# jeffreyhorn/network_flow_solver

Hardware: AMD Instinct MI355X
Metric: pivots/sec + arcs-priced/sec (value = arcs-priced/sec; pivots_per_sec alongside) on netgen_8-style DIMACS (higher is better)
Workload: dtype int64; 1 GPU; netgen_8_08a(synthetic,x1): 256 nodes / 2048 arcs; pricing=full-scan Dantzig, step=one pivot (price + ratio test + tree/potential update), parallelism=1 GPU, sweeps=full (every arc priced every pivot)

## Files before the change

__graft_entry__.py:

```python

from __future__ import annotations

import os
import re
import subprocess
import sys
from pathlib import Path

ROOT = Path(__file__).resolve().parent
PKG = ROOT / "network_flow_solver_amd"
CSRC = PKG / "csrc"
LIB = PKG / "libmcf_hip.so"
CERT_HOST_LIB = PKG / "libmcf_certify_host.so"
REPAIR_HOST_LIB = PKG / "libmcf_repair_host.so"
FARKAS_HOST_LIB = PKG / "libmcf_farkas_host.so"
TOPOLOGY_HOST_LIB = PKG / "libmcf_topology_host.so"
RANGES_HOST_LIB = PKG / "libmcf_ranges_host.so"
FLOW_RANGES_HOST_LIB = PKG / "libmcf_flow_ranges_host.so"
DUAL_HOST_LIB = PKG / "libmcf_dual_host.so"
APPLY_PATHS_HOST_LIB = PKG / "libmcf_apply_paths_host.so"
SMALL_REDUCE_HOST_LIB = PKG / "libmcf_small_reduce_host.so"

if str(ROOT) not in sys.path:
    sys.path.insert(0, str(ROOT))


def _hipcc() -> str:
    for cand in (os.environ.get("HIPCC"), "/opt/rocm/bin/hipcc", "hipcc"):
        if cand and (os.path.isabs(cand) and os.path.exists(cand) or not os.path.isabs(cand)):
            return cand
    return "hipcc"


def _needs_rebuild(target: Path, sources) -> bool:
    if not target.exists():
        return True
    t = target.stat().st_mtime
    return any(Path(s).stat().st_mtime > t for s in sources)


def build_hip(force: bool = False) -> Path:
    sources = [CSRC / "mcf_engine.hip", CSRC / "mcf_passes_dev.h", CSRC / "mcf_passes_host.h", CSRC / "mcf_core.h", CSRC / "mcf_host.h",
               ROOT / "include" / "mcf.h"]
    if force or _needs_rebuild(LIB, sources):
        cmd = [_hipcc(), "--offload-arch=gfx950", "-O3", "-std=c++17", "-fPIC", "-shared",
               "-o", str(LIB), str(CSRC / "mcf_engine.hip")]
        subprocess.run(cmd, check=True, cwd=str(CSRC))
    return LIB


def build_certify_host(force: bool = False) -> Path:
    src = CSRC / "mcf_certify_host.cpp"
    if force or _needs_rebuild(CERT_HOST_LIB, [src, CSRC / "mcf_core.h"]):
        subprocess.run(["g++", "-O2", "-std=c++17", "-fPIC", "-shared", "-o", str(CERT_HOST_LIB), str(src)], check=True, cwd=str(CSRC))
    return CERT_HOST_LIB


def build_repair_host(force: bool = False) -> Path:
    src = CSRC / "mcf_repair_host.cpp"
    if force or _needs_rebuild(REPAIR_HOST_LIB, [src, CSRC / "mcf_core.h", CSRC / "mcf_host.h"]):
        subprocess.run(["g++", "-O2", "-std=c++17", "-fPIC", "-shared", "-o", str(REPAIR_HOST_LIB), str(src)], check=True, cwd=str(CSRC))
    return REPAIR_HOST_LIB


def build_farkas_host(force: bool = False) -> Path:
    src = CSRC / "mcf_farkas_host.cpp"
    if force or _needs_rebuild(FARKAS_HOST_LIB, [src, CSRC / "mcf_core.h"]):
        subprocess.run(["g++", "-O2", "-std=c++17", "-fPIC", "-shared", "-o", str(FARKAS_HOST_LIB), str(src)], check=True, cwd=str(CSRC))
    return FARKAS_HOST_LIB


def build_topology_host(force: bool = False) -> Path:
    src = CSRC / "mcf_topology_host.cpp"
    if force or _needs_rebuild(TOPOLOGY_HOST_LIB, [src, CSRC / "mcf_core.h", CSRC / "mcf_host.h"]):
        subprocess.run(["g++", "-O2", "-std=c++17", "-fPIC", "-shared", "-o", str(TOPOLOGY_HOST_LIB), str(src)], check=True, cwd=str(CSRC))
    return TOPOLOGY_HOST_LIB


def build_ranges_host(force: bool = False) -> Path:
    src = CSRC / "mcf_ranges_host.cpp"
    if force or _needs_rebuild(RANGES_HOST_LIB, [src, CSRC / "mcf_core.h"]):
        subprocess.run(["g++", "-O2", "-std=c++17", "-fPIC", "-shared", "-o", str(RANGES_HOST_LIB), str(src)], check=True, cwd=str(CSRC))
    return RANGES_HOST_LIB


def build_flow_ranges_host(force: bool = False) -> Path:
    src = CSRC / "mcf_flow_ranges_host.cpp"
    if force or _needs_rebuild(FLOW_RANGES_HOST_LIB, [src, CSRC / "mcf_core.h"]):
        subprocess.run(["g++", "-O2", "-std=c++17", "-fPIC", "-shared", "-o", str(FLOW_RANGES_HOST_LIB), str(src)], check=True, cwd=str(CSRC))
    return FLOW_RANGES_HOST_LIB


def build_dual_host(force: bool = False) -> Path:
    src = CSRC / "mcf_dual_host.cpp"
    if force or _needs_rebuild(DUAL_HOST_LIB, [src, CSRC / "mcf_core.h", CSRC / "mcf_host.h", ROOT / "include" / "mcf.h"]):
        subprocess.run(["g++", "-O2", "-std=c++17", "-fPIC", "-shared", "-o", str(DUAL_HOST_LIB), str(src)], check=True, cwd=str(CSRC))
    return DUAL_HOST_LIB


def build_apply_paths_host(force: bool = False) -> Path:
    src = CSRC / "mcf_apply_paths_host.cpp"
    if force or _needs_rebuild(APPLY_PATHS_HOST_LIB, [src, CSRC / "mcf_core.h", CSRC / "mcf_host.h"]):
        subprocess.run(["g++", "-O2", "-std=c++17", "-fPIC", "-shared", "-o", str(APPLY_PATHS_HOST_LIB), str(src)], check=True, cwd=str(CSRC))
    return APPLY_PATHS_HOST_LIB


def build_small_reduce_host(force: bool = False) -> Path:
    src = CSRC / "mcf_small_reduce_host.cpp"
    if force or _needs_rebuild(SMALL_REDUCE_HOST_LIB, [src, CSRC / "mcf_core.h"]):
        subprocess.run(["g++", "-O2", "-std=c++17", "-fPIC", "-shared", "-o", str(SMALL_REDUCE_HOST_LIB), str(src)], check=True, cwd=str(CSRC))
    return SMALL_REDUCE_HOST_LIB


def declared_symbols() -> list[str]:
    text = (ROOT / "include" / "mcf.h").read_text()
    text = re.sub(r"/\*.*?\*/", "", text, flags=re.S)
    names = re.findall(r"\b(mcf_[a-z0-9_]+)\s*\(", text)
    return sorted(set(n for n in names if n != "mcf_progress_cb"))


def build() -> None:
    build_hip()
    import oracle

    oracle.build()
    oracle.build_emul()
    build_certify_host()
    build_repair_host()
    build_farkas_host()
    build_topology_host()
    build_ranges_host()
    build_flow_ranges_host()
    build_dual_host()
    build_apply_paths_host()
    build_small_reduce_host()
    import ctypes

    lib = ctypes.CDLL(str(LIB))
    missing = [s for s in declared_symbols() if not hasattr(lib, s)]
    if missing:
        raise RuntimeError(f"libmcf_hip.so lacks symbols declared in include/mcf.h: {missing}")
    import network_flow_solver_amd


def smoke() -> None:
    import numpy as np

    build_hip()
    import oracle
    from network_flow_solver_amd import engine, generators

    if engine.device_count() <= 0:
        raise RuntimeError("smoke() needs a GPU: no HIP device visible")
    inst = generators.netgen_style(256, 2048, seed=7)
    ref = oracle.solve_soa(inst, "dantzig")
    for rule in (engine.RULE_DANTZIG, engine.RULE_DEVEX_BLOCK, engine.RULE_CANDIDATE_LIST):
        with engine.McfEngine(inst.n, inst.tail, inst.head, inst.cost, inst.cap, inst.supply, rule=rule,
                              device=0) as eng:
            eng.solve()
            res = eng.result()
        assert res.status == ref["status"] == "optimal", (res.status, ref["status"])
        assert res.objective == int(round(ref["objective"])), (res.objective, ref["objective"])
        bal = inst.supply.astype(np.int64).copy()
        np.subtract.at(bal, inst.tail, res.flow)
        np.add.at(bal, inst.head, res.flow)
        assert not bal.any()
        rc = inst.cost + res.potential[inst.tail] - res.potential[inst.head]
        assert (rc[(res.flow > 0) & (res.flow < inst.cap)] == 0).all()
        assert (rc[(res.flow == 0) & (inst.cap > 0)] >= 0).all() and (rc[(res.flow == inst.cap) & (inst.cap > 0)] <= 0).all()
        print(f"smoke ok: rule={rule} objective={res.objective} pivots={res.stats['pivots']} "
              f"(oracle {ref['iterations']} pivots)")


if __name__ == "__main__":
    build()
    if len(sys.argv) > 1 and sys.argv[1] == "smoke":
        smoke()
```

network_flow_solver_amd/csrc/mcf_core.h:

```cpp
#pragma once
#include <stdint.h>

#if defined(__HIPCC__)
#define MCF_HD __host__ __device__ __forceinline__
#else
#define MCF_HD inline
#endif

#define MCF_INF ((int64_t)1 << 60)

#if defined(__HIP_DEVICE_COMPILE__)
#define mcf_double_bits(x) ((int64_t)__double_as_longlong(x))
#else
static inline int64_t mcf_double_bits(double x) { int64_t k; __builtin_memcpy(&k, &x, 8); return k; }
#endif

#if defined(__HIP_DEVICE_COMPILE__)
#define MCF_TEAM_BARRIER() __syncthreads()
#define MCF_ATOMIC_MIN64(p, x) atomicMin(reinterpret_cast<long long*>(p), (long long)(x))
#define MCF_ATOMIC_MIN32(p, x) atomicMin(reinterpret_cast<int*>(p), (int)(x))
#define MCF_ATOMIC_MAX32(p, x) atomicMax(reinterpret_cast<int*>(p), (int)(x))
#define MCF_ATOMIC_ADD32(p, x) atomicAdd(reinterpret_cast<int*>(p), (int)(x))
#define MCF_ATOMIC_MAX64(p, x) atomicMax(reinterpret_cast<long long*>(p), (long long)(x))
#define MCF_ATOMIC_OR32(p, x) atomicOr(reinterpret_cast<int*>(p), (int)(x))
// ... 6 lines not shown
#define MCF_ATOMIC_ADD32(p, x) mcf_host_fetch_add32((p), (x))
#define MCF_ATOMIC_MAX64(p, x) do { if ((int64_t)(x) > *(p)) *(p) = (int64_t)(x); } while (0)
#define MCF_ATOMIC_OR32(p, x) do { *(p) |= (int32_t)(x); } while (0)
#endif

enum McfStatus : int32_t {
    MCF_RUNNING = 0,
    MCF_OPTIMAL = 1,
    MCF_PIVOT_LIMIT = 2,
    MCF_UNBOUNDED = 3,
    MCF_INTERNAL_ERROR = 4
};

#define MCF_RULE_DANTZIG 0
#ifndef MCF_RULE_DEVEX_BLOCK
#define MCF_RULE_DEVEX_BLOCK 1
#endif
#ifndef MCF_RULE_CANDIDATE_LIST
#define MCF_RULE_CANDIDATE_LIST 2
#endif

#if defined(__HIPCC__)
template <int CTRL, int ROW_MASK>
__device__ __forceinline__ int64_t mcf_dpp_max_step(int64_t x) {
    const int lo = (int)(uint32_t)x, hi = (int)(uint32_t)((uint64_t)x >> 32);
    const int olo = __builtin_amdgcn_update_dpp(lo, lo, CTRL, ROW_MASK, 0xf, false);
    const int ohi = __builtin_amdgcn_update_dpp(hi, hi, CTRL, ROW_MASK, 0xf, false);
    const int64_t o = (int64_t)(((uint64_t)(uint32_t)ohi << 32) | (uint32_t)olo);
    return o > x ? o : x;
}
__device__ __forceinline__ int64_t mcf_wave_max64(int64_t x) {
    x = mcf_dpp_max_step<0xB1, 0xf>(x);
    x = mcf_dpp_max_step<0x4E, 0xf>(x);
    x = mcf_dpp_max_step<0x141, 0xf>(x);
    x = mcf_dpp_max_step<0x140, 0xf>(x);
    x = mcf_dpp_max_step<0x142, 0xa>(x);
    x = mcf_dpp_max_step<0x143, 0xc>(x);
    const uint32_t lo = (uint32_t)__builtin_amdgcn_readlane((int)(uint32_t)x, 63);
    const uint32_t hi = (uint32_t)__builtin_amdgcn_readlane((int)(uint32_t)((uint64_t)x >> 32), 63);
    return (int64_t)(((uint64_t)hi << 32) | lo);
}
template <int CTRL, int ROW_MASK>
__device__ __forceinline__ uint32_t mcf_dpp_min_u32_step(uint32_t x) {
    const uint32_t o = (uint32_t)__builtin_amdgcn_update_dpp((int)0xffffffffu, (int)x, CTRL, ROW_MASK, 0xf, false);
    return o < x ? o : x;
}
template <int CTRL, int ROW_MASK>
__device__ __forceinline__ uint32_t mcf_dpp_max_u32_step(uint32_t x) {
    const uint32_t o = (uint32_t)__builtin_amdgcn_update_dpp(0, (int)x, CTRL, ROW_MASK, 0xf, false);
    return o > x ? o : x;
}
__device__ __forceinline__ uint32_t mcf_wave_min_u32(uint32_t x) {
    x = mcf_dpp_min_u32_step<0xB1, 0xf>(x);
    x = mcf_dpp_min_u32_step<0x4E, 0xf>(x);
    x = mcf_dpp_min_u32_step<0x141, 0xf>(x);
    x = mcf_dpp_min_u32_step<0x140, 0xf>(x);
    x = mcf_dpp_min_u32_step<0x142, 0xa>(x);
    x = mcf_dpp_min_u32_step<0x143, 0xc>(x);
    return (uint32_t)__builtin_amdgcn_readlane((int)x, 63);
}
__device__ __forceinline__ uint32_t mcf_wave_max_u32(uint32_t x) {
    x = mcf_dpp_max_u32_step<0xB1, 0xf>(x);
    x = mcf_dpp_max_u32_step<0x4E, 0xf>(x);
    x = mcf_dpp_max_u32_step<0x141, 0xf>(x);
    x = mcf_dpp_max_u32_step<0x140, 0xf>(x);
    x = mcf_dpp_max_u32_step<0x142, 0xa>(x);
    x = mcf_dpp_max_u32_step<0x143, 0xc>(x);
    return (uint32_t)__builtin_amdgcn_readlane((int)x, 63);
}
#endif

MCF_HD bool mcf_ratio_narrow_ok(int64_t r) { return r == MCF_INF || (uint64_t)r <= 0xfffffffeull; }
MCF_HD uint32_t mcf_ratio_key32(int64_t r) { return r == MCF_INF ? 0xffffffffu : (uint32_t)r; }
MCF_HD int64_t mcf_ratio_unkey32(uint32_t k) { return k == 0xffffffffu ? MCF_INF : (int64_t)k; }
template <bool LAST>
MCF_HD void mcf_ratio_take(int64_t mn, uint64_t mask, int32_t base, int64_t& d, int32_t& k) {
    if (LAST ? mn <= d : mn < d) {
        d = mn;
        k = base + (LAST ? 63 - __builtin_clzll((unsigned long long)mask) : __builtin_ctzll((unsigned long long)mask));
    }
}
MCF_HD uint32_t mcf_argmax_viol(uint64_t packed) { return (uint32_t)(packed >> 32); }
MCF_HD uint32_t mcf_argmax_second(uint64_t packed, uint32_t vmx) { return mcf_argmax_viol(packed) == vmx ? (uint32_t)packed : 0u; }

#if defined(MCF_STAMPS) && defined(__HIPCC__)
__shared__ unsigned long long mcf_stamp_acc[24];
__shared__ unsigned long long mcf_stamp_last;
#define MCF_PSTAMP(slot)                                                     \
    do {                                                                      \
        if (threadIdx.x == 0) {                                               \
            const unsigned long long now_ = __builtin_amdgcn_s_memtime();     \
            mcf_stamp_acc[slot] += now_ - mcf_stamp_last;                     \
            mcf_stamp_last = now_;                                            \
        }                                                                     \
    } while (0)
#else
#define MCF_PSTAMP(slot) do {} while (0)
#endif

struct alignas(16) McfNode {
    int32_t parent;
    int32_t pred;
    int32_t size;
    int32_t depth;
};

struct alignas(16) McfArcW {
    int64_t cap;
    int64_t flow;
};

struct alignas(16) McfCand {
    int64_t key;
    int64_t arc;
};

struct alignas(16) McfCandX {
    int64_t rc;
    int64_t arc;
    int32_t tail, head;
    int32_t state;
    int32_t pad;
};

#define MCF_NUM_BUCKETS 8

#define MCF_GRANULES 64
#define MCF_WLIST_CAP 1024
#define MCF_DEVEX_RESET_SWAPS 64
#define MCF_TUNER_MAX_ARCS 16384
#define MCF_DIR_FLAG (1 << 30)
struct McfDevex {
    int32_t gran[MCF_NUM_BUCKETS][MCF_GRANULES + 1];
    int32_t gtot[MCF_GRANULES + 1];
    int32_t wlist[MCF_WLIST_CAP];
};

struct McfSeg {
    int32_t dst, src, len;
    int32_t ddepth;
};

struct McfCtx {
    int32_t status;
    int32_t unbounded_arc;
    int64_t pivots;
    int64_t degenerate;
    int64_t bound_flips;
    int64_t max_pivots;
    int64_t arcs_priced;
    int64_t nodes_moved;
    int64_t subtree_nodes;
    int64_t cycle_arcs;
    int64_t block_size;
    int64_t block_index;
    int32_t empty_blocks;
    int32_t num_blocks;
    int32_t block_granules;
    int32_t auto_tune;
    int32_t tn_total, tn_degenerate;
    int64_t tn_last_adapt;
    int32_t swaps_since_reset;
    int32_t wlist_n;
    int32_t wreset;
    int32_t devex_cyclic;
    int32_t max_granules;
// ... 1850 lines not shown
```

network_flow_solver_amd/csrc/mcf_engine.hip:

```cpp
#include <hip/hip_runtime.h>

#include <algorithm>
#include <cerrno>
#include <chrono>
#include <cstdio>
#include <cstdlib>
#include <cstring>
#include <mutex>
#include <new>
#include <string>
#include <vector>

#include "../../include/mcf.h"
#include "mcf_core.h"
#include "mcf_host.h"

namespace {

constexpr int kPriceThreads = 256;
constexpr int kPivotThreads = 1024;
constexpr int kReduceThreads = 256;
constexpr int kMidMaxNodes = 1536;
constexpr int kMidMaxArcsPerPivot = MCF_TUNER_MAX_ARCS + 1024;
constexpr int64_t kIncrementalMinArcs = (int64_t)1 << 22;
// ... 1200 lines not shown
template <bool MARK>
__global__ __launch_bounds__(kRcupdThreads) void k_rcupd(McfView g) {
    McfView v = g;
    if (!MARK) v.dirty = nullptr;
    const McfCtx c = *v.ctx;
    if (!c.apply) return;
    rcupd_pass(v, c, (int64_t)blockIdx.x * (kRcupdThreads / 16) + (threadIdx.x >> 4), (int64_t)gridDim.x * (kRcupdThreads / 16), threadIdx.x & 15);
}

__global__ __launch_bounds__(kApplyThreads) void k_apply(McfView v) {
    const McfCtx c = *v.ctx;
    if (!c.apply) return;
    const int xb = v.candx ? kCandxBlocks : 0;
    const int nb = (int)gridDim.x - xb;
    if ((int)blockIdx.x >= nb) { candx_pass(v, c, ((int)blockIdx.x - nb) * kApplyThreads + (int)threadIdx.x, xb * kApplyThreads); return; }
    apply_pass(v, c, (int64_t)blockIdx.x * kApplyThreads + threadIdx.x, (int64_t)nb * kApplyThreads);
}

__device__ __forceinline__ int swap01(int x) { return __builtin_amdgcn_update_dpp(x, x, 0xB1, 0xf, 0xf, false); }

__device__ __forceinline__ bool pivot_climb_2lanes(const McfView& v, McfCycle* out) {
    const McfCtx* c = v.ctx;
    const int side = threadIdx.x & 1;
    const int32_t* pcur = c->cur ? v.posbuf[1] : v.posbuf[0];
    int32_t node = side ? c->pv_second : c->pv_first;
    McfNode rec = v.node[node];
    int32_t pos = pcur[node];
    const McfNode rec0 = rec;
    const int32_t pos0 = pos;
    int32_t* const path = side ? v.path2 : v.path1;
    int32_t* const ppos = side ? v.ppos2 : v.ppos1;
    McfNode* const recs = side ? v.rec2 : v.rec1;
    int64_t d = MCF_INF;
    int32_t k = -1, n = 0, trips = 0;
    bool ok = true;
    for (;;) {
        const int32_t onode = swap01(node), odepth = swap01(rec.depth);
        if (node == onode) break;
        if (rec.depth >= odepth) {
            const McfNode nrec = v.node[rec.parent];
            const int32_t npos = pcur[rec.parent];
            const McfArcW a = v.arcw[rec.pred >> 1];
            const bool loses = ((rec.pred & 1) != 0) != (side != 0);
            const int64_t r = loses ? a.flow : (a.cap >= MCF_INF ? MCF_INF : a.cap - a.flow);
            if (side ? r <= d : r < d) { d = r; k = n; }
            path[n] = node;
            recs[n] = rec;
            ppos[n] = pos;
            ++n;
            node = rec.parent;
            rec = nrec;
            pos = npos;
        }
        if (++trips > v.n_nodes) { ok = false; break; }
    }
    const int32_t od_lo = swap01((int)(uint32_t)d), od_hi = swap01((int)(uint32_t)((uint64_t)d >> 32));
    const int32_t ok2 = swap01(k), on2 = swap01(n), opos0 = swap01(pos0);
    McfNode orec0;
    orec0.parent = swap01(rec0.parent); orec0.pred = swap01(rec0.pred); orec0.size = swap01(rec0.size); orec0.depth = swap01(rec0.depth);
    if (side == 0) {
        out->d1 = d; out->k1 = k; out->n1 = n;
        out->d2 = (int64_t)(((uint64_t)(uint32_t)od_hi << 32) | (uint32_t)od_lo); out->k2 = ok2; out->n2 = on2;
        out->u = node; out->w = node; out->pu = pos; out->pw = pos; out->ru = rec; out->rw = rec;
        out->p0u = pos0; out->p0w = opos0; out->r0u = rec0; out->r0w = orec0;
        out->small = 0;
    }
    return ok;
}

struct SmallLayout {
    uint32_t tail, head, cost, orig, state, weight, arcw, pi, node, order0, order1, pos0, pos1, path1, path2, ppos1, ppos2, rec1, rec2, seg, scratch, ctx, total;
};

constexpr int kSmallMaxLds = 156 * 1024;
constexpr int kSmallCycleMaxNodes = 1024;

#if defined(MCF_SMALL_LDS_SWEEP)
constexpr bool kRegSweep = false;
#else
constexpr bool kRegSweep = true;
#endif
template <int THREADS> struct SmallScalarControl { static constexpr bool value = THREADS > 256; };
template <int THREADS> struct SmallRegArcs { static constexpr int value = THREADS <= 256 ? 10 : (THREADS <= 512 ? 5 : 3); };

template <int THREADS>
__device__ __forceinline__ void copy_words(void* dst, const void* src, uint32_t bytes) {
    const uint32_t n = bytes >> 2;
    const int32_t* s = static_cast<const int32_t*>(src);
    int32_t* d = static_cast<int32_t*>(dst);
    for (uint32_t i = threadIdx.x; i < n; i += THREADS) d[i] = s[i];
}

#ifdef MCF_STAMPS
#define STAMP(slot)                                                                       \
    do {                                                                                  \
        if (threadIdx.x == 0) {                                                           \
            const unsigned long long now_ = __builtin_amdgcn_s_memtime();                 \
            stamps_[slot] += now_ - last_;                                                \
            last_ = now_;                                                                 \
        }                                                                                 \
    } while (0)
#else
#define STAMP(slot) do {} while (0)
#endif
#ifdef MCF_STAMPS
#define MCF_LAST_WAVE_BEGIN() const unsigned long long lw0_ = __builtin_amdgcn_s_memtime()
#define MCF_LAST_WAVE_STAMP() do { last_wave_ += __builtin_amdgcn_s_memtime() - lw0_; } while (0)
#else
#define MCF_LAST_WAVE_BEGIN() do {} while (0)
#define MCF_LAST_WAVE_STAMP() do {} while (0)
#endif

struct SmallCycleAcc {
    int32_t c1[16], c2[16];
};
#if defined(MCF_SMALL_JOIN)
template <int THREADS> struct SmallSearchJoin { static constexpr bool value = true; };
#else
template <int THREADS> struct SmallSearchJoin { static constexpr bool value = THREADS != 256; };
#endif

#if defined(MCF_SMALL_RATIO64)
constexpr bool kRatioNarrow = false;
#else
constexpr bool kRatioNarrow = true;
#endif
template <bool LAST>
__device__ __forceinline__ void small_ratio_side(const int64_t* res, int32_t n, int64_t* d_out, int32_t* k_out) {
    const int32_t lane = (int32_t)(threadIdx.x & 63);
    int64_t d = MCF_INF;
    int32_t k = -1;
    if (kRatioNarrow) {
        const int64_t r0 = lane < n ? res[lane] : MCF_INF;
        bool wide = !mcf_ratio_narrow_ok(r0);
        for (int32_t i = 64 + lane; i < n; i += 64) wide |= !mcf_ratio_narrow_ok(res[i]);
        if (__ballot(wide) == 0) {
            for (int32_t base = 0; base < n; base += 64) {
                const int32_t i = base + lane;
                const uint32_t key = mcf_ratio_key32(base == 0 ? r0 : (i < n ? res[i] : MCF_INF));
                const uint32_t mn = mcf_wave_min_u32(key);
                const uint64_t mask = __ballot(i < n && key == mn);
                mcf_ratio_take<LAST>(mcf_ratio_unkey32(mn), mask, base, d, k);
            }
            *d_out = d; *k_out = k;
            return;
        }
    }
    for (int32_t base = 0; base < n; base += 64) {
        const int32_t i = base + lane;
        const int64_t r = i < n ? res[i] : INT64_MAX;
        const int64_t mn = -mcf_wave_max64(-r);
        const uint64_t mask = __ballot(r == mn);
        mcf_ratio_take<LAST>(mn, mask, base, d, k);
    }
    *d_out = d; *k_out = k;
}

#if defined(MCF_SMALL_TWO_BRANCHES)
template <int THREADS> struct SmallSearchOneBranch { static constexpr bool value = false; };
#else
template <int THREADS> struct SmallSearchOneBranch { static constexpr bool value = THREADS == 256; };
#endif

template <int THREADS>
__device__ __forceinline__ void small_cycle_parallel(const McfView& v, SmallCycleAcc& A, int64_t* scratch, McfCycle& cy) {
    constexpr bool kScalar = SmallScalarControl<THREADS>::value;
// ... 262 lines not shown
    const uint32_t m_padb = m_pad4 >> 2;
    const uint32_t N = (uint32_t)g.n_nodes;
    const uint32_t arcw_b = (uint32_t)(g.m + N - 1) * 16u;
    McfView v = g;
    v.tail = reinterpret_cast<const int32_t*>(smem + L.tail);
    v.head = reinterpret_cast<const int32_t*>(smem + L.head);
    v.cost = reinterpret_cast<const int32_t*>(smem + L.cost);
    v.orig = reinterpret_cast<const int32_t*>(smem + L.orig);
    v.state = reinterpret_cast<int8_t*>(smem + L.state);
    v.weight = g.weight ? reinterpret_cast<float*>(smem + L.weight) : nullptr;
    v.arcw = reinterpret_cast<McfArcW*>(smem + L.arcw);
    v.pi = reinterpret_cast<int64_t*>(smem + L.pi);
    v.node = reinterpret_cast<McfNode*>(smem + L.node);
    v.order[0] = reinterpret_cast<int32_t*>(smem + L.order0);
    v.order[1] = reinterpret_cast<int32_t*>(smem + L.order1);
    v.path1 = reinterpret_cast<int32_t*>(smem + L.path1);
    v.path2 = reinterpret_cast<int32_t*>(smem + L.path2);
    v.ppos1 = reinterpret_cast<int32_t*>(smem + L.ppos1);
    v.ppos2 = reinterpret_cast<int32_t*>(smem + L.ppos2);
    v.rec1 = reinterpret_cast<McfNode*>(smem + L.rec1);
    v.rec2 = reinterpret_cast<McfNode*>(smem + L.rec2);
    v.seg = reinterpret_cast<McfSeg*>(smem + L.seg);
    v.ctx = reinterpret_cast<McfCtx*>(smem + L.ctx);
    v.posbuf[0] = reinterpret_cast<int32_t*>(smem + L.pos0);
    v.posbuf[1] = reinterpret_cast<int32_t*>(smem + L.pos1);
    v.psz[0] = nullptr;
    v.psz[1] = nullptr;
    v.reach = nullptr;
    v.bmeta[0] = nullptr; v.bmeta[1] = nullptr; v.candx = nullptr; v.dirty = nullptr; v.dirty_hdr = nullptr;
    v.rcache = nullptr; v.adj_off = nullptr;
    if constexpr (FRONT && kFrontNoDevex) { v.weight = nullptr; v.dx = nullptr; }

    copy_words<THREADS>(smem + L.tail, g.tail, m_pad4);
    copy_words<THREADS>(smem + L.head, g.head, m_pad4);
    copy_words<THREADS>(smem + L.cost, g.cost, m_pad4);
    copy_words<THREADS>(smem + L.orig, g.orig, m_pad4);
    copy_words<THREADS>(smem + L.state, g.state, m_padb);
    if (v.weight) copy_words<THREADS>(smem + L.weight, g.weight, m_pad4);
    copy_words<THREADS>(smem + L.arcw, g.arcw, arcw_b);
    copy_words<THREADS>(smem + L.pi, g.pi, N * 8u);
    copy_words<THREADS>(smem + L.node, g.node, N * 16u);
    copy_words<THREADS>(smem + L.order0, g.order[0], N * 4u);
    copy_words<THREADS>(smem + L.order1, g.order[1], N * 4u);
    copy_words<THREADS>(smem + L.pos0, g.posbuf[0], N * 4u);
    copy_words<THREADS>(smem + L.pos1, g.posbuf[1], N * 4u);
    copy_words<THREADS>(smem + L.ctx, g.ctx, (uint32_t)sizeof(McfCtx));
    __syncthreads();
    STAMP(0);

    McfCtx* const c = v.ctx;
    if (threadIdx.x == 0) arm_ctx(c, cap);
    __shared__ int32_t s_gran[MCF_NUM_BUCKETS][MCF_GRANULES + 1];
    const bool devex = !FRONT && rule == MCF_RULE_DEVEX_BLOCK && g.dx;
    if (devex) {
        for (int q = threadIdx.x; q < MCF_NUM_BUCKETS * (MCF_GRANULES + 1); q += THREADS)
            (&s_gran[0][0])[q] = (&g.dx->gran[0][0])[q];
    } else if (threadIdx.x < MCF_NUM_BUCKETS) {
        s_gran[threadIdx.x][0] = (int32_t)g.bucket_off[threadIdx.x];
        s_gran[threadIdx.x][MCF_GRANULES] = (int32_t)g.bucket_off[threadIdx.x + 1];
    }
    const bool listing = !FRONT && rule == MCF_RULE_CANDIDATE_LIST;
    __shared__ int64_t s_lk[MCF_NUM_BUCKETS], s_la[MCF_NUM_BUCKETS];
    if (listing && threadIdx.x < MCF_NUM_BUCKETS) { s_lk[threadIdx.x] = list[threadIdx.x].key; s_la[threadIdx.x] = list[threadIdx.x].arc; }
    __syncthreads();
    __shared__ int32_t s_gsum[MCF_GRANULES + 1];
    if (threadIdx.x <= MCF_GRANULES && (devex || threadIdx.x == 0 || threadIdx.x == MCF_GRANULES)) {
        int32_t sum = 0;
        for (int x = 0; x < MCF_NUM_BUCKETS; ++x) sum += s_gran[x][threadIdx.x];
        s_gsum[threadIdx.x] = sum;
    }
    __syncthreads();
    constexpr bool kScalar = SmallScalarControl<THREADS>::value;
    const int64_t priced_all = uni32<kScalar>(s_gsum[MCF_GRANULES] - s_gsum[0]);

    constexpr int kPer = THREADS / MCF_NUM_BUCKETS;
    constexpr int kReg = SmallRegArcs<THREADS>::value;
    static_assert(kPer == 32 || kPer % 64 == 0, "a head bucket's lanes are half a wave or whole waves");
    const int px = threadIdx.x / kPer, pl = threadIdx.x % kPer;
    const int sweep = FRONT ? (int)kSweepPlain
                            : (devex ? kSweepDevex : (rule != MCF_RULE_DEVEX_BLOCK && v.key_mode == MCF_KEY_PLAIN ? kSweepPlain : kSweepGeneric));
    int32_t r_tail[kReg], r_head[kReg], r_cost[kReg], r_orig[kReg];
    uint32_t r_info[kReg];
    int32_t r_n = 0;
    const int32_t r_lo = s_gran[px][0] + pl, r_hi = s_gran[px][MCF_GRANULES];
#pragma unroll
    for (int k = 0; k < kReg; ++k) {
        const int32_t i = r_lo + k * kPer;
        const bool on = kRegSweep && sweep == kSweepPlain && i < r_hi;
        r_tail[k] = on ? v.tail[i] : 0; r_head[k] = on ? v.head[i] : 0; r_cost[k] = on ? v.cost[i] : 0; r_orig[k] = on ? v.orig[i] : 0;
        r_info[k] = small_info(r_tail[k], r_head[k], k);
        r_n += on ? 1 : 0;
    }
    const bool reg_plain = kRegSweep && sweep == kSweepPlain;
    constexpr bool nar = FRONT;
    constexpr bool kDescOnce = SmallDescOnce<THREADS, FRONT>::value;
    constexpr bool hand = FRONT && kHandover;
    const int32_t* const pi32 = reinterpret_cast<const int32_t*>(v.pi);
    McfCtx cx = *c;
    small_ctx_uniform<kScalar>(cx);
    cx.max_pivots = uni64<kScalar>(cx.max_pivots); cx.minor_cap = uni32<kScalar>(cx.minor_cap); cx.auto_tune = uni32<kScalar>(cx.auto_tune);
    cx.devex_cyclic = uni32<kScalar>(cx.devex_cyclic); cx.max_granules = uni32<kScalar>(cx.max_granules);
    v.ctx = &cx;
    const int64_t adj2 = uni64<kScalar>(cx.pv_adj[2]), adj3 = uni64<kScalar>(cx.pv_adj[3]);
    int64_t* const scratch = reinterpret_cast<int64_t*>(smem + L.scratch);
    __shared__ McfCycle s_cy;
    __shared__ int s_ok;
    __shared__ SmallCycleAcc s_acc;
    for (;;) {
        if (cx.status != MCF_RUNNING) break;
        const bool minor = listing && cx.minor_left > 0;
        int32_t bg0 = 0, bg1 = MCF_GRANULES;
        if (devex) {
            const int32_t bg = cx.block_granules;
            bg0 = (int32_t)cx.block_index * bg;
            if (bg0 >= MCF_GRANULES) bg0 = 0;
            bg1 = bg0 + bg < MCF_GRANULES ? bg0 + bg : MCF_GRANULES;
        }
        int64_t key = 0, arc = -1;
        McfCandX wx;
        wx.rc = 0; wx.arc = -1; wx.tail = 0; wx.head = 0; wx.state = 0; wx.pad = 0;
        uint64_t nbest = 0xffffffffull;
        uint32_t info = 0;
        if (!minor) {
            if (nar) {
                int32_t st[kReg], pt[kReg], ph[kReg];
#pragma unroll
                for (int k = 0; k < kReg; ++k) {
                    st[k] = v.state[k < r_n ? r_lo + k * kPer : 0];
                    pt[k] = pi32[2 * r_tail[k]];
                    ph[k] = pi32[2 * r_head[k]];
                }
#pragma unroll
                for (int k = 0; k < kReg; ++k) {
                    const int32_t rc = (int32_t)((uint32_t)r_cost[k] + (uint32_t)pt[k] - (uint32_t)ph[k]);
                    const int32_t s = k < r_n ? st[k] : 0;
                    const int32_t viol = s > 0 ? -rc : rc;
                    const uint64_t p = ((uint64_t)(uint32_t)((s != 0 && viol > 0) ? viol : 0) << 32) | (uint32_t)~r_orig[k];
                    if (p > nbest) { nbest = p; info = r_info[k] | ((uint32_t)s & 0x80000000u); }
                }
                int32_t q = kReg;
                for (int32_t i = r_lo + kReg * kPer; i < r_hi; i += kPer, ++q) small_price_lds_narrow(v, i, q, nbest, info);
                if (nbest >> 32) { key = (int64_t)(nbest >> 32); arc = mcf_pack_arc((int32_t)~(uint32_t)nbest, r_lo + (int32_t)((info >> 22) & 0x1ff) * kPer); }
            } else if (reg_plain) {
                int32_t st[kReg];
                int64_t pt[kReg], ph[kReg];
#pragma unroll
                for (int k = 0; k < kReg; ++k) {
                    st[k] = v.state[k < r_n ? r_lo + k * kPer : 0];
                    pt[k] = v.pi[r_tail[k]];
                    ph[k] = v.pi[r_head[k]];
                }
#pragma unroll
                for (int k = 0; k < kReg; ++k) {
                    const int64_t rc = (int64_t)r_cost[k] + pt[k] - ph[k];
                    const int32_t s = k < r_n ? st[k] : 0;
                    const int64_t viol = s > 0 ? -rc : rc;
                    const int64_t pid = mcf_pack_arc(r_orig[k], r_lo + k * kPer);
                    if (s != 0 && viol > 0 && mcf_cand_better(viol, pid, key, arc)) { key = viol; arc = pid; }
                }
                for (int32_t i = r_lo + kReg * kPer; i < r_hi; i += kPer) small_price_lds<kSweepPlain>(v, rule, devex, i, key, arc);
            } else {
                const int32_t lo = s_gran[px][bg0], hi = s_gran[px][bg1];
                if (sweep == kSweepDevex) for (int32_t i = lo + pl; i < hi; i += kPer) small_price_lds<kSweepDevex>(v, rule, devex, i, key, arc);
                else if (sweep == kSweepPlain) for (int32_t i = lo + pl; i < hi; i += kPer) small_price_lds<kSweepPlain>(v, rule, devex, i, key, arc);
                else for (int32_t i = lo + pl; i < hi; i += kPer) small_price_lds<kSweepGeneric>(v, rule, devex, i, key, arc);
            }
        }
        STAMP(1);
        if (listing) {
            if (!minor) {
                if constexpr (kPer >= 64) {
                    constexpr int kWpb = kPer / 64;
                    __shared__ int64_t s_wk[THREADS / 64], s_wa[THREADS / 64];
                    wave_argmax(key, arc);
                    if ((threadIdx.x & 63) == 0) { s_wk[threadIdx.x >> 6] = key; s_wa[threadIdx.x >> 6] = arc; }
                    __syncthreads();
                    if (threadIdx.x < MCF_NUM_BUCKETS) {
                        const int w = kWpb * threadIdx.x;
                        int64_t bk = s_wk[w], ba = s_wa[w];
                        for (int q = 1; q < kWpb; ++q)
                            if (mcf_cand_better(s_wk[w + q], s_wa[w + q], bk, ba)) { bk = s_wk[w + q]; ba = s_wa[w + q]; }
                        s_lk[threadIdx.x] = bk; s_la[threadIdx.x] = ba;
                    }
                } else {
                    half_wave_argmax(key, arc);
                    if (pl == 0) { s_lk[px] = key; s_la[px] = arc; }
                }
                __syncthreads();
            }
            const int32_t l = (int32_t)(threadIdx.x & 63);
            key = 0; arc = -1;
            if (l < MCF_NUM_BUCKETS) {
                arc = s_la[l];
                key = minor ? mcf_minor_key(v, arc) : s_lk[l];
                if (key <= 0) { key = 0; arc = -1; }
            }
            wave_argmax(key, arc);
        } else if (hand) {
            constexpr int kWaves = THREADS / 64;
            __shared__ SmallWaveSlot s_slot[kWaves];
            const int32_t lane = (int32_t)(threadIdx.x & 63), wave = (int32_t)(threadIdx.x >> 6);
            bool any, win;
            if constexpr (kArgmaxStaged) {
                const uint32_t vmx = mcf_wave_max_u32(mcf_argmax_viol(nbest));
                any = vmx != 0;
                win = mcf_argmax_viol(nbest) == vmx;
                const uint64_t tied = __ballot(win);
                if (any && (tied & (tied - 1))) {
                    const uint32_t imx = mcf_wave_max_u32(mcf_argmax_second(nbest, vmx));
                    win = win && (uint32_t)nbest == imx;
                }
            } else {
                const uint64_t mx = (uint64_t)mcf_wave_max64((int64_t)nbest);
                any = (mx >> 32) != 0;
                win = nbest == mx;
            }
            if (any ? win : lane == 0) s_slot[wave] = SmallWaveSlot{any ? nbest : 0, (int32_t)(arc & 0xffffffff), info};
            __syncthreads();
            SmallWaveSlot b;
            if constexpr (kWaves <= 4) {
                SmallWaveSlot sl[kWaves];
#pragma unroll
                for (int q = 0; q < kWaves; ++q) sl[q] = s_slot[q];
                b = sl[0];
#pragma unroll
                for (int q = 1; q < kWaves; ++q) if (sl[q].key > b.key) b = sl[q];
            } else {
                const SmallWaveSlot mine = s_slot[lane < kWaves ? lane : 0];
                const uint64_t k = lane < kWaves ? mine.key : 0;
                b.key = (uint64_t)mcf_wave_max64((int64_t)k);
                const int32_t w = (int32_t)__builtin_ctzll((unsigned long long)__ballot(k == b.key));
                b.e = __builtin_amdgcn_readlane(mine.e, w);
                b.info = (uint32_t)__builtin_amdgcn_readlane((int32_t)mine.info, w);
            }
            key = (int64_t)(b.key >> 32);
            if (key > 0) {
                wx = small_record(b.info, key, (int32_t)~(uint32_t)b.key, b.e);
                arc = wx.arc;
            } else { key = 0; arc = -1; }
            key = uni64<kScalar>(key); arc = uni64<kScalar>(arc);
            wx.rc = uni64<kScalar>(wx.rc); wx.tail = uni32<kScalar>(wx.tail); wx.head = uni32<kScalar>(wx.head); wx.state = uni32<kScalar>(wx.state);
        } else {
            block_argmax_all<THREADS>(key, arc);
// ... 1898 lines not shown
```

Measured before the change: 610.1 million arcs/s.

## Deal small-kernel register arcs evenly across all threads and shorten the unrolled sweep

In the small single-block kernel's Dantzig plain sweep, register-resident arcs are now dealt round-robin across all threads (stride THREADS from the global start) instead of per-bucket strides. This balances the per-thread arc count. When the arcs fit in fewer slots, a shorter unrolled pricing loop (8 instead of 10 slots) is instantiated to cut masked work and register pressure. The change also adds a host-side checker library for the dealing arithmetic, and it risks altering the bucket-local structure that later listing or reduction steps may assume.

```diff
diff --git a/__graft_entry__.py b/__graft_entry__.py
--- a/__graft_entry__.py
+++ b/__graft_entry__.py
@@ -20,6 +20,7 @@
 DUAL_HOST_LIB = PKG / "libmcf_dual_host.so"
 APPLY_PATHS_HOST_LIB = PKG / "libmcf_apply_paths_host.so"
 SMALL_REDUCE_HOST_LIB = PKG / "libmcf_small_reduce_host.so"
+SMALL_CYCLE_REGS_HOST_LIB = PKG / "libmcf_small_cycle_regs_host.so"
 
 if str(ROOT) not in sys.path:
     sys.path.insert(0, str(ROOT))
@@ -112,6 +113,13 @@
     return SMALL_REDUCE_HOST_LIB
 
 
+def build_small_cycle_regs_host(force: bool = False) -> Path:
+    src = CSRC / "mcf_small_cycle_regs_host.cpp"
+    if force or _needs_rebuild(SMALL_CYCLE_REGS_HOST_LIB, [src, CSRC / "mcf_core.h"]):
+        subprocess.run(["g++", "-O2", "-std=c++17", "-fPIC", "-shared", "-o", str(SMALL_CYCLE_REGS_HOST_LIB), str(src)], check=True, cwd=str(CSRC))
+    return SMALL_CYCLE_REGS_HOST_LIB
+
+
 def declared_symbols() -> list[str]:
     text = (ROOT / "include" / "mcf.h").read_text()
     text = re.sub(r"/\*.*?\*/", "", text, flags=re.S)
@@ -134,6 +142,7 @@
     build_dual_host()
     build_apply_paths_host()
     build_small_reduce_host()
+    build_small_cycle_regs_host()
     import ctypes
 
     lib = ctypes.CDLL(str(LIB))
diff --git a/network_flow_solver_amd/csrc/mcf_core.h b/network_flow_solver_amd/csrc/mcf_core.h
--- a/network_flow_solver_amd/csrc/mcf_core.h
+++ b/network_flow_solver_amd/csrc/mcf_core.h
@@ -112,6 +112,12 @@
 }
 MCF_HD uint32_t mcf_argmax_viol(uint64_t packed) { return (uint32_t)(packed >> 32); }
 MCF_HD uint32_t mcf_argmax_second(uint64_t packed, uint32_t vmx) { return mcf_argmax_viol(packed) == vmx ? (uint32_t)packed : 0u; }
+
+MCF_HD int32_t mcf_even_arc(int32_t base, int32_t lane, int32_t slot, int32_t threads) { return base + lane + slot * threads; }
+MCF_HD int32_t mcf_even_slots(int32_t arcs, int32_t threads) { return (arcs + threads - 1) / threads; }
+MCF_HD int32_t mcf_even_reg_slots(int32_t arcs, int32_t threads, int32_t few, int32_t reg) {
+    return mcf_even_slots(arcs, threads) <= few ? few : reg;
+}
 
 #if defined(MCF_STAMPS) && defined(__HIPCC__)
 __shared__ unsigned long long mcf_stamp_acc[24];
diff --git a/network_flow_solver_amd/csrc/mcf_engine.hip b/network_flow_solver_amd/csrc/mcf_engine.hip
--- a/network_flow_solver_amd/csrc/mcf_engine.hip
+++ b/network_flow_solver_amd/csrc/mcf_engine.hip
@@ -1306,6 +1306,23 @@
 #endif
 template <int THREADS> struct SmallScalarControl { static constexpr bool value = THREADS > 256; };
 template <int THREADS> struct SmallRegArcs { static constexpr int value = THREADS <= 256 ? 10 : (THREADS <= 512 ? 5 : 3); };
+template <int THREADS, bool FRONT> struct SmallEvenDeal {
+#if defined(MCF_SMALL_BUCKET_DEAL)
+    static constexpr bool value = false;
+#elif defined(MCF_SMALL_EVEN_GENERAL)
+    static constexpr bool value = true;
+#else
+    static constexpr bool value = FRONT;
+#endif
+};
+#if defined(MCF_SMALL_EVEN_ALL_SLOTS)
+template <int THREADS, bool FRONT> struct SmallRegArcsFew { static constexpr int value = SmallRegArcs<THREADS>::value; };
+#else
+template <int THREADS, bool FRONT> struct SmallRegArcsFew {
+    static constexpr int value = !FRONT ? SmallRegArcs<THREADS>::value : (THREADS <= 256 ? 8 : (THREADS <= 512 ? 4 : 2));
+};
+#endif
+template <int N> struct SmallSlots { static constexpr int value = N; };
 
 template <int THREADS>
 __device__ __forceinline__ void copy_words(void* dst, const void* src, uint32_t bytes) {
@@ -1734,10 +1751,16 @@
     int32_t r_tail[kReg], r_head[kReg], r_cost[kReg], r_orig[kReg];
     uint32_t r_info[kReg];
     int32_t r_n = 0;
-    const int32_t r_lo = s_gran[px][0] + pl, r_hi = s_gran[px][MCF_GRANULES];
+    constexpr int kRegFew = SmallRegArcsFew<THREADS, FRONT>::value;
+    static_assert(kRegFew <= kReg, "the shorter unrolled sweep is a prefix of the longer");
+    const bool even = SmallEvenDeal<THREADS, FRONT>::value && kRegSweep && sweep == kSweepPlain && rule == MCF_RULE_DANTZIG;
+    const int32_t r_step = even ? THREADS : kPer;
+    const int32_t r_lo = even ? mcf_even_arc(s_gran[0][0], (int32_t)threadIdx.x, 0, THREADS) : s_gran[px][0] + pl;
+    const int32_t r_hi = even ? s_gran[MCF_NUM_BUCKETS - 1][MCF_GRANULES] : s_gran[px][MCF_GRANULES];
+    const bool r_few = even && uni32<kScalar>(mcf_even_reg_slots(s_gran[MCF_NUM_BUCKETS - 1][MCF_GRANULES] - s_gran[0][0], THREADS, kRegFew, kReg)) == kRegFew;
 #pragma unroll
     for (int k = 0; k < kReg; ++k) {
-        const int32_t i = r_lo + k * kPer;
+        const int32_t i = r_lo + k * r_step;
         const bool on = kRegSweep && sweep == kSweepPlain && i < r_hi;
         r_tail[k] = on ? v.tail[i] : 0; r_head[k] = on ? v.head[i] : 0; r_cost[k] = on ? v.cost[i] : 0; r_orig[k] = on ? v.orig[i] : 0;
         r_info[k] = small_info(r_tail[k], r_head[k], k);
@@ -1775,42 +1798,52 @@
         uint32_t info = 0;
         if (!minor) {
             if (nar) {
-                int32_t st[kReg], pt[kReg], ph[kReg];
+                auto slots = [&](auto ns) {
+                    constexpr int NS = decltype(ns)::value;
+                    int32_t st[NS], pt[NS], ph[NS];
 #pragma unroll
-                for (int k = 0; k < kReg; ++k) {
-                    st[k] = v.state[k < r_n ? r_lo + k * kPer : 0];
-                    pt[k] = pi32[2 * r_tail[k]];
-                    ph[k] = pi32[2 * r_head[k]];
-                }
+                    for (int k = 0; k < NS; ++k) {
+                        st[k] = v.state[k < r_n ? r_lo + k * r_step : 0];
+                        pt[k] = pi32[2 * r_tail[k]];
+                        ph[k] = pi32[2 * r_head[k]];
+                    }
 #pragma unroll
-                for (int k = 0; k < kReg; ++k) {
-                    const int32_t rc = (int32_t)((uint32_t)r_cost[k] + (uint32_t)pt[k] - (uint32_t)ph[k]);
-                    const int32_t s = k < r_n ? st[k] : 0;
-                    const int32_t viol = s > 0 ? -rc : rc;
-                    const uint64_t p = ((uint64_t)(uint32_t)((s != 0 && viol > 0) ? viol : 0) << 32) | (uint32_t)~r_orig[k];
-                    if (p > nbest) { nbest = p; info = r_info[k] | ((uint32_t)s & 0x80000000u); }
-                }
+                    for (int k = 0; k < NS; ++k) {
+                        const int32_t rc = (int32_t)((uint32_t)r_cost[k] + (uint32_t)pt[k] - (uint32_t)ph[k]);
+                        const int32_t s = k < r_n ? st[k] : 0;
+                        const int32_t viol = s > 0 ? -rc : rc;
+                        const uint64_t p = ((uint64_t)(uint32_t)((s != 0 && viol > 0) ? viol : 0) << 32) | (uint32_t)~r_orig[k];
+                        if (p > nbest) { nbest = p; info = r_info[k] | ((uint32_t)s & 0x80000000u); }
+                    }
+                };
+                if (r_few) slots(SmallSlots<kRegFew>{});
+                else slots(SmallSlots<kReg>{});
                 int32_t q = kReg;
-                for (int32_t i = r_lo + kReg * kPer; i < r_hi; i += kPer, ++q) small_price_lds_narrow(v, i, q, nbest, info);
-                if (nbest >> 32) { key = (int64_t)(nbest >> 32); arc = mcf_pack_arc((int32_t)~(uint32_t)nbest, r_lo + (int32_t)((info >> 22) & 0x1ff) * kPer); }
+                for (int32_t i = r_lo + kReg * r_step; i < r_hi; i += r_step, ++q) small_price_lds_narrow(v, i, q, nbest, info);
+                if (nbest >> 32) { key = (int64_t)(nbest >> 32); arc = mcf_pack_arc((int32_t)~(uint32_t)nbest, r_lo + (int32_t)((info >> 22) & 0x1ff) * r_step); }
             } else if (reg_plain) {
-                int32_t st[kReg];
-                int64_t pt[kReg], ph[kReg];
+                auto slots = [&](auto ns) {
+                    constexpr int NS = decltype(ns)::value;
+                    int32_t st[NS];
+                    int64_t pt[NS], ph[NS];
 #pragma unroll
-                for (int k = 0; k < kReg; ++k) {
-                    st[k] = v.state[k < r_n ? r_lo + k * kPer : 0];
-                    pt[k] = v.pi[r_tail[k]];
-                    ph[k] = v.pi[r_head[k]];
-                }
+                    for (int k = 0; k < NS; ++k) {
+                        st[k] = v.state[k < r_n ? r_lo + k * r_step : 0];
+                        pt[k] = v.pi[r_tail[k]];
+                        ph[k] = v.pi[r_head[k]];
+                    }
 #pragma unroll
-                for (int k = 0; k < kReg; ++k) {
-                    const int64_t rc = (int64_t)r_cost[k] + pt[k] - ph[k];
-                    const int32_t s = k < r_n ? st[k] : 0;
-                    const int64_t viol = s > 0 ? -rc : rc;
-                    const int64_t pid = mcf_pack_arc(r_orig[k], r_lo + k * kPer);
-                    if (s != 0 && viol > 0 && mcf_cand_better(viol, pid, key, arc)) { key = viol; arc = pid; }
-                }
-                for (int32_t i = r_lo + kReg * kPer; i < r_hi; i += kPer) small_price_lds<kSweepPlain>(v, rule, devex, i, key, arc);
+                    for (int k = 0; k < NS; ++k) {
+                        const int64_t rc = (int64_t)r_cost[k] + pt[k] - ph[k];
+                        const int32_t s = k < r_n ? st[k] : 0;
+                        const int64_t viol = s > 0 ? -rc : rc;
+                        const int64_t pid = mcf_pack_arc(r_orig[k], r_lo + k * r_step);
+                        if (s != 0 && viol > 0 && mcf_cand_better(viol, pid, key, arc)) { key = viol; arc = pid; }
+                    }
+                };
+                if (r_few) slots(SmallSlots<kRegFew>{});
+                else slots(SmallSlots<kReg>{});
+                for (int32_t i = r_lo + kReg * r_step; i < r_hi; i += r_step) small_price_lds<kSweepPlain>(v, rule, devex, i, key, arc);
             } else {
                 const int32_t lo = s_gran[px][bg0], hi = s_gran[px][bg1];
                 if (sweep == kSweepDevex) for (int32_t i = lo + pl; i < hi; i += kPer) small_price_lds<kSweepDevex>(v, rule, devex, i, key, arc);
diff --git a/network_flow_solver_amd/csrc/mcf_small_cycle_regs_driver.cpp b/network_flow_solver_amd/csrc/mcf_small_cycle_regs_driver.cpp
--- /dev/null
+++ b/network_flow_solver_amd/csrc/mcf_small_cycle_regs_driver.cpp
@@ -0,0 +1,31 @@
+#include <cstdint>
+#include <cstdio>
+#include <cstdlib>
+#include <vector>
+
+extern "C" int mcf_small_even_deal_host(int32_t base, int32_t arcs, int32_t threads, int32_t few, int32_t reg, int32_t* times,
+                                        int32_t* lane_of, int32_t* slot_of, int32_t* from_lds, int32_t* slots_out, int64_t* masked_out);
+
+int main(int argc, char** argv) {
+    if ((argc - 1) % 5 != 0) { std::fprintf(stderr, "five numbers per case\n"); return 2; }
+    int bad = 0;
+    for (int a = 1; a + 4 < argc; a += 5) {
+        const int32_t base = (int32_t)std::atol(argv[a]), arcs = (int32_t)std::atol(argv[a + 1]), threads = (int32_t)std::atol(argv[a + 2]);
+        const int32_t few = (int32_t)std::atol(argv[a + 3]), reg = (int32_t)std::atol(argv[a + 4]);
+        if (arcs < 0 || arcs > (1 << 24)) return 2;
+        std::vector<int32_t> times((size_t)arcs, 0), lane((size_t)arcs, -1), slot((size_t)arcs, -1), lds((size_t)arcs, -1);
+        int32_t slots = 0;
+        int64_t masked = 0;
+        if (mcf_small_even_deal_host(base, arcs, threads, few, reg, times.data(), lane.data(), slot.data(), lds.data(), &slots, &masked) != 0) {
+            bad = 1;
+            continue;
+        }
+        int64_t from_lds = 0;
+        for (int32_t i = 0; i < arcs; ++i) {
+            if (times[(size_t)i] != 1 || lane[(size_t)i] != i % threads) bad = 1;
+            from_lds += lds[(size_t)i];
+        }
+        std::printf("%d %lld %lld %d\n", slots, (long long)masked, (long long)from_lds, arcs ? slot[(size_t)arcs - 1] : -1);
+    }
+    return bad;
+}
diff --git a/network_flow_solver_amd/csrc/mcf_small_cycle_regs_host.cpp b/network_flow_solver_amd/csrc/mcf_small_cycle_regs_host.cpp
--- /dev/null
+++ b/network_flow_solver_amd/csrc/mcf_small_cycle_regs_host.cpp
@@ -0,0 +1,37 @@
+#include <cstdint>
+
+#include "mcf_core.h"
+
+extern "C" {
+
+int mcf_small_even_deal_host(int32_t base, int32_t arcs, int32_t threads, int32_t few, int32_t reg, int32_t* times, int32_t* lane_of,
+                             int32_t* slot_of, int32_t* from_lds, int32_t* slots_out, int64_t* masked_out) {
+    if (base < 0 || arcs < 0 || threads <= 0 || few <= 0 || few > reg || !slots_out || !masked_out) return -1;
+    if (arcs > 0 && (!times || !lane_of || !slot_of || !from_lds)) return -1;
+    const int32_t r_hi = base + arcs;
+    const int32_t ns = mcf_even_reg_slots(arcs, threads, few, reg);
+    int64_t masked = 0;
+    for (int32_t t = 0; t < threads; ++t) {
+        const int32_t r_lo = mcf_even_arc(base, t, 0, threads);
+        int32_t r_n = 0;
+        for (int32_t k = 0; k < reg; ++k) r_n += mcf_even_arc(base, t, k, threads) < r_hi ? 1 : 0;
+        for (int32_t k = 0; k < ns; ++k) {
+            if (!(k < r_n)) { ++masked; continue; }
+            const int32_t i = mcf_even_arc(base, t, k, threads);
+            if (i < base || i >= r_hi || r_lo + k * threads != i) return -2;
+            times[i - base] += 1; lane_of[i - base] = t; slot_of[i - base] = k; from_lds[i - base] = 0;
+        }
+        int32_t q = reg;
+        for (int32_t i = r_lo + reg * threads; i < r_hi; i += threads, ++q) {
+            if (i < base || r_lo + q * threads != i) return -2;
+            times[i - base] += 1; lane_of[i - base] = t; slot_of[i - base] = q; from_lds[i - base] = 1;
+        }
+    }
+    *slots_out = ns;
+    *masked_out = masked;
+    return 0;
+}
+
+int32_t mcf_small_even_slots_host(int32_t arcs, int32_t threads) { return mcf_even_slots(arcs, threads); }
+
+}
```

Result: faster. 624.7 million arcs/s (median of 6 runs) (+2.4%).
